# ntnu-arl/aerial_gym_simulator

Hardware: AMD Instinct MI355X
Metric: env-steps/sec at N_envs=8192 per GPU (dynamics-only) (higher is better)
Workload: dtype f32; 1 GPU; base_quadrotor position_setpoint_task, lee_position_control, empty_env, 1 sub-step/step (BASELINE configs[1]); num_envs_per_gpu=8192, num_envs_total=8192, rng=sync-free (device Philox4x32-10)

## Files before the change

aerial_gym_simulator_amd/csrc/agx_dyn_position_step.h:

```cpp
#pragma once

namespace agx {
#ifdef AGX_STEP_STAMPS
constexpr int kStampBlocks = 1024, kStampWords = 8;
__device__ unsigned long long g_step_stamps[kStampBlocks * 2 * kStampWords];
AGX_DEV void step_stamp(int k) {
  const unsigned long long t = k < 6 ? (unsigned long long)clock64() : (unsigned long long)wall_clock64();
  if ((threadIdx.x & 63u) == 0u && blockIdx.x < (unsigned)kStampBlocks)
    g_step_stamps[((size_t)blockIdx.x * 2 + (threadIdx.x >> 6)) * kStampWords + k] = t;
}
#define AGX_STAMP(k) step_stamp(k)
#define AGX_STAMP_ARRIVED(k) do { __builtin_amdgcn_s_waitcnt(0); step_stamp(k); } while (0)
#else
#define AGX_STAMP(k) do { } while (0)
#define AGX_STAMP_ARRIVED(k) do { } while (0)
#endif

AGX_DEV unsigned proof_key(float x) { return x >= 0.0f ? __float_as_uint(x) : 0x7FC00000u; }

__host__ __device__ inline unsigned proof_witness_bit(int episode_len, int reset_on_collision, int steps, float dist, float speed, float dt,
                                                      float vmax, float dv) {
  const int k = episode_len - steps + 1;
  if (k < 1 || k > AGX_PROOF_HORIZON || !(dist == dist) || !(speed == speed)) return 0u;
  bool w = k == 1 || !reset_on_collision;
  if (!w) {
    const float m = (float)(k - 1);
    const float travel = m * dt * fminf(vmax, speed + m * dv);
    w = dist + (travel * 1.01f + 1.0e-3f) < 8.0f;
  }
  return w ? (1u << k) : 0u;
}

template <bool MAX>
AGX_DEV unsigned wave_reduce_dpp(unsigned x) {
#define AGX_RED(ctrl)                                                                        \
  {                                                                                           \
    const unsigned y_ = (unsigned)__builtin_amdgcn_mov_dpp((int)x, (ctrl), 0xF, 0xF, true);   \
    x = MAX ? max(x, y_) : (x | y_);                                                          \
  }
  AGX_RED(0xB1)
  AGX_RED(0x4E)
  AGX_RED(0x124)
  AGX_RED(0x128)
#undef AGX_RED
  const unsigned r0 = (unsigned)__builtin_amdgcn_readlane((int)x, 0), r1 = (unsigned)__builtin_amdgcn_readlane((int)x, 16);
  const unsigned r2 = (unsigned)__builtin_amdgcn_readlane((int)x, 32), r3 = (unsigned)__builtin_amdgcn_readlane((int)x, 48);
  return MAX ? max(max(r0, r1), max(r2, r3)) : ((r0 | r1) | (r2 | r3));
}

AGX_DEV void proof_store_slot(const AgxTaskArgs &T, const AgxEnvBuffers &B, int wb, int nb, bool reset, unsigned horizon, int steps,
                              float dist, float speed) {
  const unsigned ar = wave_reduce_dpp<false>(reset ? 1u : 0u), hz = wave_reduce_dpp<false>(horizon);
  const unsigned ms = wave_reduce_dpp<true>((unsigned)max(steps, 0)), db = wave_reduce_dpp<true>(proof_key(dist));
  const unsigned vb = wave_reduce_dpp<true>(proof_key(speed));
  if ((threadIdx.x & 63u) == 0u) {
    uint4 *slot = reinterpret_cast<uint4 *>(T.proof_slots + ((size_t)(B.step_counter & 1) * nb + wb) * AGX_PROOF_SLOT_WORDS);
    slot[0] = make_uint4(((unsigned)B.step_counter + 1u) & 0x7FFFFFFFu, ar | (T.proof_mode == AGX_STEP_ANY ? 2u : 0u), hz, ms);
    slot[1] = make_uint4(db, vb, 0u, 0u);
  }
}

AGX_DEV void proof_fold_publish(const AgxTaskArgs &T, const AgxEnvBuffers &B, int nb) {
  const int lane = (int)(threadIdx.x & 63u);
  const uint32_t *bank = T.proof_slots + (size_t)((B.step_counter & 1) ^ 1) * nb * AGX_PROOF_SLOT_WORDS;
  unsigned t_and = 0x7FFFFFFFu, t_or = 0u, fl = 0u, hz = 0u, ms = 0u, db = 0u, vb = 0u;
  for (int b = lane; b < nb; b += 64) {
    const uint4 s0 = reinterpret_cast<const uint4 *>(bank + (size_t)b * AGX_PROOF_SLOT_WORDS)[0];
    const uint4 s1 = reinterpret_cast<const uint4 *>(bank + (size_t)b * AGX_PROOF_SLOT_WORDS)[1];
    t_and &= s0.x; t_or |= s0.x; fl |= s0.y; hz |= s0.z;
    ms = max(ms, s0.w); db = max(db, s1.x); vb = max(vb, s1.y);
  }
#pragma unroll
  for (int off = 32; off > 0; off >>= 1) {
    t_and &= (unsigned)__shfl_xor((int)t_and, off);
    t_or |= (unsigned)__shfl_xor((int)t_or, off);
    fl |= (unsigned)__shfl_xor((int)fl, off);
    hz |= (unsigned)__shfl_xor((int)hz, off);
    ms = max(ms, (unsigned)__shfl_xor((int)ms, off));
    db = max(db, (unsigned)__shfl_xor((int)db, off));
    vb = max(vb, (unsigned)__shfl_xor((int)vb, off));
  }
  if (lane != 0) return;
  const unsigned tag = t_and == t_or ? t_or : 0u;
  if (tag != 0u && (fl & 2u) && !(fl & 1u)) atomicAdd(T.proof_violation, 1u);
  uint32_t *h = T.proof_record;
  __hip_atomic_store(h + 7, tag, __ATOMIC_RELAXED, __HIP_MEMORY_SCOPE_SYSTEM);
  __builtin_amdgcn_fence(__ATOMIC_RELEASE, "wavefront");
  __builtin_amdgcn_s_waitcnt(0);
  __hip_atomic_store(h + 1, hz, __ATOMIC_RELAXED, __HIP_MEMORY_SCOPE_SYSTEM);
  __hip_atomic_store(h + 2, ms, __ATOMIC_RELAXED, __HIP_MEMORY_SCOPE_SYSTEM);
  __hip_atomic_store(h + 3, db, __ATOMIC_RELAXED, __HIP_MEMORY_SCOPE_SYSTEM);
  __hip_atomic_store(h + 4, vb, __ATOMIC_RELAXED, __HIP_MEMORY_SCOPE_SYSTEM);
  __hip_atomic_store(h + 5, fl, __ATOMIC_RELAXED, __HIP_MEMORY_SCOPE_SYSTEM);
  __builtin_amdgcn_fence(__ATOMIC_RELEASE, "wavefront");
  __builtin_amdgcn_s_waitcnt(0);
  __hip_atomic_store(h + 0, tag, __ATOMIC_RELAXED, __HIP_MEMORY_SCOPE_SYSTEM);
}

struct StepHandoff {
  float p[64], q[64], v[64], w[64];
  int reset[64];
};
template <int MODE>
AGX_DEV void position_step_quad(const AgxRobotParams &P0, const AgxEnvBuffers &B0, int n, const float *actions_in,
                                const AgxTaskArgs &T0, float *obs, StepHandoff *H) {
  constexpr bool FUSED = MODE != AGX_STEP_TWO;
  const int tid = threadIdx.x;
  AGX_STAMP(0); AGX_STAMP(6);
  AgxRobotParams P = P0;
  AgxEnvBuffers B = B0;
  AgxTaskArgs T = T0;
#define AGX_STEP_WAVE_ARGS(X)                                                                                                        \
  X(B, state) X(B, actions) X(B, prev_actions) X(B, motor_thrust) X(B, motor_kT) X(B, motor_tau_inc) X(B, motor_tau_dec)  \
  X(B, gains) X(B, wrench_cmd) X(B, crashes) X(B, truncations) X(B, sim_steps) X(B, reset_mask) X(B, reset_flag) X(B, flag_parity)    \
  X(B, step_counter) X(B, body_force)                                                                                                  \
  X(P, dt) X(P, dt_over_6) X(P, mass) X(P, min_thrust) X(P, max_thrust) X(P, max_rate) X(P, linear_damping) X(P, angular_damping)     \
  X(P, max_linear_velocity) X(P, max_angular_velocity) X(P, tau_inc_uniform) X(P, tau_dec_uniform)                                    \
  X(T, episode_len) X(T, target) X(T, reward) X(T, proof_slots) X(T, proof_violation) X(T, proof_dv)
  AGX_STEP_WAVE_ARGS(AGX_ARG_READ)
  AGX_ARG_READ(B, derived) AGX_ARG_READ(B, push_world)
  AGX_ARG_READ(P, root_link_mode) AGX_ARG_READ(P, use_rps) AGX_ARG_READ(P, use_discrete_approximation) AGX_ARG_READ(P, integration_rk4)
  AGX_ARG_READ(T, reset_on_collision) AGX_ARG_READ(T, kind) AGX_ARG_READ(T, proof_mode)
  const int grid_blocks = (int)gridDim.x;
  __builtin_amdgcn_sched_barrier(0);
  int env_blocks = grid_blocks - 1;
  int sw = (P_root_link_mode != 0 ? 1 : 0) | (P_use_rps != 0 ? 2 : 0) | (P_use_discrete_approximation != 0 ? 4 : 0) |
           (P_integration_rk4 != 0 ? 8 : 0) | (T_reset_on_collision != 0 ? 16 : 0) | ((T_kind & 0xFF) << 8) | ((T_proof_mode & 0xFF) << 16);
  arg_pin(n); arg_pin(actions_in);
  if (MODE == AGX_STEP_NONE) arg_pin(obs);
  AGX_STEP_WAVE_ARGS(AGX_ARG_PIN)
  if (MODE != AGX_STEP_ANY) { AGX_ARG_PIN(B, derived) }
  if (!FUSED) { AGX_ARG_PIN(B, push_world) }
  arg_pin(env_blocks);
#undef AGX_STEP_WAVE_ARGS
  arg_pin(sw);
  P.root_link_mode = sw & 1; P.use_rps = sw & 2; P.use_discrete_approximation = sw & 4; P.integration_rk4 = sw & 8;
  T.reset_on_collision = sw & 16; T.kind = (sw >> 8) & 0xFF; T.proof_mode = (sw >> 16) & 0xFF;
  const bool proof = T.proof_slots != nullptr;
  if (proof && blockIdx.x == 0) {
    proof_fold_publish(T0, B0, (int)gridDim.x - 1);
    AGX_STAMP(5); AGX_STAMP(7);
    return;
  }
  const int wb = (int)blockIdx.x - (proof ? 1 : 0);
  const int l = tid & 3, l3 = l < 3 ? l : 2;
  const int i = wb * 16 + (tid >> 2);
  const unsigned ol = ((unsigned)l * (unsigned)n + (unsigned)i) * 4u, ol3 = ((unsigned)l3 * (unsigned)n + (unsigned)i) * 4u;
  const bool valid = i < n;
  bool reset = false;
  if (FUSED && wb == 0 && tid == 0) B.reset_flag[B.flag_parity ^ 1] = 0;
  const bool push = !FUSED && wb == 0 && B.push_world > 0;
  uint32_t push_peek = 0u;
  if (__builtin_expect(push, false)) {
    push_publish_previous(B0);
    push_peek = push_wait_peek(B0);
  }
  float p = 0.0f, q = 0.0f, v = 0.0f, w = 0.0f, tgt = 0.0f, vbody = 0.0f, wbody = 0.0f;
  int steps = 0;
  float proof_dist = 0.0f, proof_speed = 0.0f;
  unsigned horizon = 0u;
  float u[1] = {0.0f}, a_in = 0.0f, a_old = 0.0f, fz = 0.0f, torque = 0.0f, dist = 0.0f;
  QuadDerived d{};
  bool crashed = false, trunc = false;
  AGX_STAMP(1);
  if (valid) {
    p = AGX_QAT(B.state, 0, ol3); q = AGX_QAT(B.state, 3, ol); v = AGX_QAT(B.state, 7, ol3); w = AGX_QAT(B.state, 10, ol3);
    u[0] = AGX_QAT(B.motor_thrust, 0, ol);
    float kT[1] = {1.0f}, tinc[1] = {P.tau_inc_uniform}, tdec[1] = {P.tau_dec_uniform};
    if (P.use_rps) kT[0] = AGX_QAT(B.motor_kT, 0, ol);
    if (B.motor_tau_inc) tinc[0] = AGX_QAT(B.motor_tau_inc, 0, ol);
    if (B.motor_tau_dec) tdec[0] = AGX_QAT(B.motor_tau_dec, 0, ol);
    a_in = actions_in[(size_t)i * 4 + l];
    a_old = AGX_QAT(B.actions, 0, ol);
    float kp = P0.gains_uniform[0 + l3], kv = P0.gains_uniform[3 + l3], kr = P0.gains_uniform[6 + l3], kw = P0.gains_uniform[9 + l3];
    if (B.gains) {
      kp = gain_load(&AGX_QAT(B.gains, 0, ol3)); kv = gain_load(&AGX_QAT(B.gains, 3, ol3));
      kr = gain_load(&AGX_QAT(B.gains, 6, ol3)); kw = gain_load(&AGX_QAT(B.gains, 9, ol3));
    }
    const int steps_in = B.sim_steps[i];
    tgt = T.kind == AGX_TASK_POSITION ? AGX_QAT(T.target, 0, ol3) : 0.0f;
    const QuadConsts<4> C = load_quad_consts<4>(P0, P, l, l3);
    AGX_STAMP_ARRIVED(2);

    const float a = clamp_minmax(a_in, -10.0f, 10.0f);
    float sy_sp, cy_sp;
    d = update_states_quad(q, v, w, q4::bc<3>(a), sy_sp, cy_sp);
    const float pe = a - p;
    const float ve = 0.0f - v;
    const float acc = kp * pe + kv * ve;
    const float f = (acc - C.grav) * C.mass;
    fz = quad_thrust_along_body_z(q, f, l);
    const float qd = quad_desired_orientation_pos_vel_sc(f, sy_sp, cy_sp, l);
    torque = quad_body_torque<true>(C, q, qd, d.wbody, 0.0f, kr, kw, l);

    float fb, tb;
    quad_allocate<4>(P, C, l == 2 ? fz : 0.0f, torque, u, kT, tinc, tdec, fb, tb);
    if (B.body_force && l < 3) AGX_QAT(B.body_force, 0, ol) = fb;
    quad_integrate(P, C, p, q, v, w, fb, tb, l);

    steps = steps_in + 1;
    if (T.kind == AGX_TASK_POSITION) {
      const float pe_t = q4::quat_apply(q4::conj(d.qveh), tgt - p);
      dist = q4::norm3(pe_t);
      if (dist > 8.0f) crashed = true;
      trunc = steps > T.episode_len;
      reset = (crashed && T.reset_on_collision) || trunc;
    }
  }
  AGX_STAMP(3);
  if (MODE == AGX_STEP_ANY) {
    H->p[tid] = p; H->q[tid] = q; H->v[tid] = v; H->w[tid] = w;
    H->reset[tid] = reset ? 1 : 0;
    __syncthreads();
  }
  AGX_STAMP(4);
  if (valid) {
    float rew = 0.0f;
    if (T.kind == AGX_TASK_POSITION) {
      const float ex = exp_cw((l == 0 ? -8.0f : -4.0f) * dist * dist);
      const float pos_reward = 3.0f * q4::bc<0>(ex) + 2.0f * q4::bc<1>(ex);
      const float dist_reward = (20.0f - dist) / 40.0f;
      const float axis_z = l == 2 ? 1.0f : 0.0f;
      const float up = q4::bc<2>(q4::quat_rotate(q, axis_z));
      const float tilt = fabsf(1.0f - up);
      const float spin = q4::norm3(d.wbody);
      const float quo = (1.0f / (l == 0 ? 0.1f + tilt * tilt : 1.0f + spin * spin)) * (l == 0 ? 0.2f : 3.0f);
      const float up_reward = q4::bc<0>(quo);
      const float ang_reward = q4::bc<1>(quo);
      float total = pos_reward + dist_reward + pos_reward * (up_reward + ang_reward);
      total = 1.0f * total;
      if (crashed) total = -20.0f;
      rew = total;
      proof_dist = dist;
    }
    if (proof) {
      proof_speed = q4::norm3(v);
      if (l == 0 && !reset && T.kind == AGX_TASK_POSITION) horizon = proof_witness_bit(T.episode_len, T.reset_on_collision, steps, proof_dist, proof_speed, P.dt, P.max_linear_velocity,
                                    T.proof_dv);
    }

    const bool own = MODE != AGX_STEP_ANY || !reset;
    if (own) {
      if (l < 3) AGX_QAT(B.state, 0, ol) = p;
      AGX_QAT(B.state, 3, ol) = q;
      if (l < 3) {
        AGX_QAT(B.state, 7, ol) = v;
        AGX_QAT(B.state, 10, ol) = w;
      }
      AGX_QAT(B.motor_thrust, 0, ol) = u[0];
    }
    if (MODE != AGX_STEP_ANY) {
      if (l < 3) {
        AGX_QAT(B.derived, 0, ol) = d.euler;
        AGX_QAT(B.derived, 7, ol) = d.vveh;
        AGX_QAT(B.derived, 10, ol) = d.vbody;
        AGX_QAT(B.derived, 13, ol) = d.wbody;
      }
      AGX_QAT(B.derived, 3, ol) = d.qveh;
    }
    vbody = d.vbody;
    wbody = d.wbody;
    if (B.wrench_cmd) {
      if (l < 3) {
        AGX_QAT(B.wrench_cmd, 0, ol) = l == 2 ? fz : 0.0f;
        AGX_QAT(B.wrench_cmd, 3, ol) = torque;
      }
    }
    AGX_QAT(B.prev_actions, 0, ol) = a_old;
    AGX_QAT(B.actions, 0, ol) = a_in;
    if (l == 0) {
      if (own) B.sim_steps[i] = steps;
      if (T.kind == AGX_TASK_POSITION) {
        T.reward[i] = rew;
        B.reset_mask[i] = reset ? 1 : 0;
      }
      B.crashes[i] = crashed ? 1 : 0;
      B.truncations[i] = trunc ? 1 : 0;
    }
  }
  const bool some = __ballot(reset) != 0ull;
  if (T.kind != AGX_TASK_NONE && some && (tid & 63) == 0) {
    atomicOr(B.reset_flag + B.flag_parity, 1);
    if (MODE == AGX_STEP_NONE) atomicAdd(T.proof_violation, 1u);
  }
  if (proof) proof_store_slot(T, B, wb, env_blocks, reset, horizon, steps, proof_dist, proof_speed);
  if (!FUSED) {
    if (__builtin_expect(push, false)) push_wait_finish(B0, push_peek);
    AGX_STAMP(5); AGX_STAMP(7);
    return;
  }
  if (MODE == AGX_STEP_ANY) {
    AGX_STAMP(5); AGX_STAMP(7);
    return;
  }
  if (valid) {
    float *o = obs + (size_t)i * 13;
    const float e = tgt - p;
    if (l < 3) { o[l] = e; o[7 + l] = vbody; o[10 + l] = wbody; }
    o[3 + l] = q;
  }
  AGX_STAMP(5); AGX_STAMP(7);
}

AGX_DEV void position_step_helper(const AgxRobotParams &P0, const AgxEnvBuffers &B0, int n, const AgxTaskArgs &T0, const AgxResetArgs &R0,
                                  float *obs, const StepHandoff *H) {
  AGX_STAMP(0); AGX_STAMP(6);
  AgxRobotParams P = P0;
  AgxEnvBuffers B = B0;
  AgxTaskArgs T = T0;
  AgxResetArgs R = R0;
#define AGX_HELPER_WAVE_ARGS(X, XN)                                                                                                  \
  X(B, sim_steps) X(B, episode_count) X(B, env_index_base) X(B, bounds_min) X(B, bounds_max) X(B, state) X(B, derived) X(B, gains)    \
  X(B, motor_tau_inc) X(B, motor_tau_dec) X(B, motor_thrust) X(B, motor_kT)                                                           \
  X(P, use_rps) X(P, min_thrust) X(P, max_thrust) X(T, kind) X(T, episode_len) X(T, target) X(T, proof_slots)                         \
  XN(R, lower_bound_min, 3) XN(R, lower_bound_max, 3) XN(R, upper_bound_min, 3) XN(R, upper_bound_max, 3) XN(R, min_state, 13)        \
  XN(R, max_state, 13) XN(R, gains_min, 12) XN(R, gains_max, 12) X(R, tau_inc_min) X(R, tau_inc_max) X(R, tau_dec_min)                \
  X(R, tau_dec_max) X(R, kT_min) X(R, kT_max) X(R, randomize_gains) X(R, seed)
  AGX_HELPER_WAVE_ARGS(AGX_ARG_READ, AGX_ARG_READ_N)
  arg_pin(n); arg_pin(obs);
  AGX_HELPER_WAVE_ARGS(AGX_ARG_PIN, AGX_ARG_PIN_N)
#undef AGX_HELPER_WAVE_ARGS
  const bool proof = T.proof_slots != nullptr;
  if (proof && blockIdx.x == 0) return;
  const int lane = (int)(threadIdx.x & 63u);
  const int wb = (int)blockIdx.x - (proof ? 1 : 0);
  const int l = lane & 3, l3 = l < 3 ? l : 2;
  const int i = wb * 16 + (lane >> 2);
  const unsigned ol = ((unsigned)l * (unsigned)n + (unsigned)i) * 4u, ol3 = ((unsigned)l3 * (unsigned)n + (unsigned)i) * 4u;
  const bool valid = i < n;
  int steps_in = 0, ep = 0;
  float tgt = 0.0f;
  AGX_STAMP(1);
  if (valid) {
    steps_in = B.sim_steps[i];
    if (B.episode_count) ep = B.episode_count[i];
    tgt = T.kind == AGX_TASK_POSITION ? AGX_QAT(T.target, 0, ol3) : 0.0f;
  }
  AGX_STAMP_ARRIVED(2);
  const bool early = valid && T.kind == AGX_TASK_POSITION && steps_in + 1 > T.episode_len;
  ResetValues<4> V{};
  if (vote(early) != 0ull) {
    ResetDraws<4> D{};
    wave_reset_draws<4>(R, B.env_index_base + i, ep, early && l == 0, D);
    V = reset_env_values<4>(P, R, D);
  }
  AGX_STAMP(3);
  __syncthreads();
  AGX_STAMP(4);
  float p = H->p[lane], q = H->q[lane], v = H->v[lane], w = H->w[lane];
  const bool mine = H->reset[lane] != 0;
  const bool late = mine && !early;
  if (vote(late) != 0ull) {
    ResetDraws<4> D{};
    wave_reset_draws<4>(R, B.env_index_base + i, ep, late && l == 0, D);
    const ResetValues<4> V2 = reset_env_values<4>(P, R, D);
    if (late) V = V2;
  }
  if (vote(mine) != 0ull) {
    if (mine && l == 0) reset_env_store<4>(P, B, n, R, i, ep, V);
    const EnvState &s = V.s;
    const float npv = q4::by_lane(l3, q4::bc<0>(s.p.x), q4::bc<0>(s.p.y), q4::bc<0>(s.p.z));
    const float nq = q4::by_lane(l, q4::bc<0>(s.q.x), q4::bc<0>(s.q.y), q4::bc<0>(s.q.z), q4::bc<0>(s.q.w));
    const float nv = q4::by_lane(l3, q4::bc<0>(s.v.x), q4::bc<0>(s.v.y), q4::bc<0>(s.v.z));
    const float nw = q4::by_lane(l3, q4::bc<0>(s.w.x), q4::bc<0>(s.w.y), q4::bc<0>(s.w.z));
    p = mine ? npv : p; q = mine ? nq : q; v = mine ? nv : v; w = mine ? nw : w;
  }
  const QuadDerived d2 = update_states_quad(q, v, w);
  if (valid) {
    if (l < 3) {
      AGX_QAT(B.derived, 0, ol) = d2.euler;
      AGX_QAT(B.derived, 7, ol) = d2.vveh;
      AGX_QAT(B.derived, 10, ol) = d2.vbody;
      AGX_QAT(B.derived, 13, ol) = d2.wbody;
    }
    AGX_QAT(B.derived, 3, ol) = d2.qveh;
    float *o = obs + (size_t)i * 13;
    const float e = tgt - p;
    if (l < 3) { o[l] = e; o[7 + l] = d2.vbody; o[10 + l] = d2.wbody; }
    o[3 + l] = q;
  }
  AGX_STAMP(5); AGX_STAMP(7);
}

__global__ void __launch_bounds__(64, 1)
    k_env_step_quad_position(AgxRobotParams P, AgxEnvBuffers B, int n, const float *__restrict__ actions_in, AgxTaskArgs T) {
  position_step_quad<AGX_STEP_TWO>(P, B, n, actions_in, T, nullptr, nullptr);
}

template <int MODE>
__global__ void __launch_bounds__(MODE == AGX_STEP_ANY ? 128 : 64, 1)
    k_position_step_fused(AgxRobotParams P, AgxEnvBuffers B, int n, const float *__restrict__ actions_in, AgxTaskArgs T, AgxResetArgs R,
                          float *__restrict__ obs) {
  if constexpr (MODE == AGX_STEP_ANY) {
    __shared__ StepHandoff H;
    if (__builtin_amdgcn_readfirstlane((int)(threadIdx.x >> 6)) == 0) position_step_quad<MODE>(P, B, n, actions_in, T, obs, &H);
    else position_step_helper(P, B, n, T, R, obs, &H);
  } else {
    position_step_quad<MODE>(P, B, n, actions_in, T, obs, nullptr);
  }
}

#ifdef AGX_STEP_STAMPS
}
extern "C" int agx_debug_step_stamps(unsigned long long *out, int blocks) {
  if (blocks < 0 || blocks > agx::kStampBlocks) return -1;
  return (int)hipMemcpyFromSymbol(out, HIP_SYMBOL(agx::g_step_stamps), sizeof(unsigned long long) * 2 * agx::kStampWords * (size_t)blocks);
}
namespace agx {
#endif
}

extern "C" float agx_step_proof_dv(const AgxRobotParams *P) {
  if (!P || !(P->mass > 0.0f)) return INFINITY;
  const int M = P->num_motors;
  const float *wmap = P->root_link_mode != 0 ? P->alloc : P->wrench_map;
  float col = 0.0f;
  for (int j = 0; j < M; ++j) col += sqrtf(wmap[j] * wmap[j] + wmap[M + j] * wmap[M + j] + wmap[2 * M + j] * wmap[2 * M + j]);
  const float g = sqrtf(P->gravity[0] * P->gravity[0] + P->gravity[1] * P->gravity[1] + P->gravity[2] * P->gravity[2]);
  return (col * fmaxf(fabsf(P->max_thrust), fabsf(P->min_thrust)) / P->mass + g) * P->dt * 1.1f;
}

extern "C" float agx_step_proof_travel(int m, float speed, float dt, float vmax, float dv, int per_env) {
  if (m <= 0) return 0.0f;
  float travel = 0.0f;
  if (per_env) {
    travel = (float)m * dt * fminf(vmax, speed + (float)m * dv);
  } else {
    float v = speed;
    for (int k = 0; k < m; ++k) {
      v = fminf(v + dv, vmax);
      travel += v * dt;
    }
  }
  return travel * 1.01f + 1.0e-3f;
}

extern "C" uint32_t agx_step_proof_witness_bit(int episode_len, int reset_on_collision, int steps, float dist, float speed, float dt,
                                               float max_linear_velocity, float dv) {
  return proof_witness_bit(episode_len, reset_on_collision, steps, dist, speed, dt, max_linear_velocity, dv);
}

extern "C" int agx_step_proof_decide(const uint32_t *record, const AgxStepProofQuery *q, int32_t *reason) {
  int32_t why = AGX_PROOF_PROVED;
  int mode = AGX_STEP_TWO;
  if (!record || !q) {
    why = AGX_PROOF_OFF;
  } else {
    volatile const uint32_t *h = record;
    const uint32_t end = h[0];
    __atomic_thread_fence(__ATOMIC_ACQUIRE);
    const uint32_t hz = h[1], ms = h[2], db = h[3], vb = h[4], fl = h[5];
    __atomic_thread_fence(__ATOMIC_ACQUIRE);
    const uint32_t begin = h[7];
    const uint32_t k = (q->now_tag - end) & 0x7FFFFFFFu;
    float dist, speed;
    memcpy(&dist, &db, 4);
    memcpy(&speed, &vb, 4);
    if (end != begin) why = AGX_PROOF_TORN;
    else if (end == 0u) why = AGX_PROOF_NO_RECORD;
    else if (((end - q->min_tag) & 0x7FFFFFFFu) >= 0x40000000u) why = AGX_PROOF_VOID;
    else if (k == 0u || k > 64u) why = AGX_PROOF_TAG;
    else if (k <= AGX_PROOF_HORIZON && ((hz >> k) & 1u)) mode = AGX_STEP_ANY;
    else if (fl & 1u) why = AGX_PROOF_RESET_NO_WITNESS;
    else if ((int64_t)ms + (int64_t)k > (int64_t)q->episode_len) why = AGX_PROOF_MAY_TRUNCATE;
    else if (q->reset_on_collision && (!(speed == speed) ||
                                       !(dist + agx_step_proof_travel((int)k, speed, q->dt, q->max_linear_velocity, q->dv, 0) < 8.0f)))
      why = AGX_PROOF_MAY_CRASH;
    else mode = AGX_STEP_NONE;
  }
  if (reason) *reason = why;
  return mode;
}

extern "C" int agx_host_record_alloc(size_t bytes, void **out) {
  AGX_REQUIRE(out && bytes > 0 && bytes <= (1u << 20), "bad arguments");
  void *p = nullptr;
  const hipError_t e = hipHostMalloc(&p, bytes, hipHostMallocMapped | hipHostMallocCoherent);
  if (e != hipSuccess) return fail(AGX_E_LAUNCH, "hipHostMalloc(%zu, mapped | coherent): %s", bytes, hipGetErrorString(e));
  memset(p, 0, bytes);
  *out = p;
  return AGX_OK;
}

extern "C" int agx_host_record_free(void *p) {
  if (p) (void)hipHostFree(p);
  return AGX_OK;
}

static int position_step_mode(AgxPositionStepPlan *plan, const AgxTaskArgs &T, hipStream_t stream, bool *slots, int32_t *reason) {
  *slots = false;
  const AgxEnvBuffers *B = plan->buf;
  const AgxRobotParams *P = plan->params;
  if (!option_single_launch_step() || !plan->proof_slots || !plan->proof_record || !plan->proof_violation) {
    *reason = AGX_PROOF_OFF;
    return AGX_STEP_TWO;
  }
  const bool covered = plan->k_substeps == 1 && pick_block(plan->num_envs) == 64 && P->num_motors == 4 &&
                       P->controller == AGX_CTRL_POSITION && T.kind == AGX_TASK_POSITION && quad_kernel_usable(P, B, &T) &&
                       plan->reset->u_state == nullptr && B->episode_count && !B->step_rows[0] && !B->step_rows[1] &&
                       !B->step_signal && B->push_world <= 0 && !B->step_counter_dev && plan->obs && plan->target == T.target;
  if (!covered) {
    *reason = AGX_PROOF_NOT_COVERED;
    return AGX_STEP_TWO;
  }
  if (!plan->captured) {
    hipStreamCaptureStatus cs = hipStreamCaptureStatusNone;
    if (hipStreamIsCapturing(stream, &cs) != hipSuccess || cs != hipStreamCaptureStatusNone) plan->captured = 1;
  }
  if (plan->captured) {
    *reason = AGX_PROOF_CAPTURE;
    return AGX_STEP_TWO;
  }
  *slots = true;
  const int max_lag = plan->max_lag > 0 ? plan->max_lag : 8;
  AgxStepProofQuery Q{};
  Q.now_tag = ((uint32_t)B->step_counter + 1u) & 0x7FFFFFFFu;
  Q.min_tag = plan->proof_min_tag;
  Q.episode_len = T.episode_len;
  Q.reset_on_collision = T.reset_on_collision;
  Q.dt = P->dt;
  Q.max_linear_velocity = P->max_linear_velocity;
  Q.dv = T.proof_dv;
  if (plan->slot_run > max_lag) {
    volatile const uint32_t *h = plan->proof_record;
    uint32_t k = (Q.now_tag - h[0]) & 0x7FFFFFFFu;
    if (h[0] != 0u && k > (uint32_t)max_lag && k <= 64u) {
      const auto t0 = std::chrono::steady_clock::now();
      const auto waited = [&] {
        plan->lag_waits += 1;
        plan->lag_wait_ns += (uint64_t)std::chrono::duration_cast<std::chrono::nanoseconds>(std::chrono::steady_clock::now() - t0).count();
      };
      for (unsigned spin = 1;; ++spin) {
        k = (Q.now_tag - h[0]) & 0x7FFFFFFFu;
        if (k <= (uint32_t)max_lag || k > 64u) break;
        __builtin_ia32_pause();
        if ((spin & 255u) == 0u && std::chrono::steady_clock::now() - t0 > std::chrono::microseconds(2000)) {
          waited();
          *reason = AGX_PROOF_LAG;
          return AGX_STEP_TWO;
        }
      }
      waited();
    }
  }
  return agx_step_proof_decide(plan->proof_record, &Q, reason);
}

extern "C" int agx_position_task_step(AgxPositionStepPlan *plan, const float *actions_in, void *stream) {
  AGX_REQUIRE(plan && plan->params && plan->buf && plan->task && plan->reset, "null plan member");
  AGX_REQUIRE(plan->max_lag == 0 || (plan->max_lag >= 2 && plan->max_lag < AGX_PROOF_HORIZON), "max_lag %d outside 2 .. %d (0: 8)",
              plan->max_lag, AGX_PROOF_HORIZON - 1);
  plan->buf->flag_parity ^= 1;
  if (plan->buf->push_world > 0)
    if (int e = agx_push_advance(plan->buf)) return e;
  AgxTaskArgs T = *plan->task;
  T.proof_slots = nullptr;
  T.proof_record = nullptr;
  T.proof_violation = nullptr;
  T.proof_mode = AGX_STEP_TWO;
  T.proof_dv = agx_step_proof_dv(plan->params);
  bool slots = false;
  int32_t why = AGX_PROOF_OFF;
  const int mode = position_step_mode(plan, T, (hipStream_t)stream, &slots, &why);
  plan->last_mode = mode;
  plan->last_reason = why;
  plan->mode_count[mode] += 1;
  plan->reason_count[why] += 1;
  plan->slot_run = slots ? plan->slot_run + 1 : 0;
  if (slots) {
    T.proof_slots = plan->proof_slots;
    T.proof_record = plan->proof_record;
    T.proof_violation = plan->proof_violation;
    T.proof_mode = mode;
  }
  if (mode != AGX_STEP_TWO) {
    const AgxEnvBuffers *B = plan->buf;
    const int n = plan->num_envs;
    if (int e = check_reset(plan->params, B, n, plan->reset)) return e;
    AGX_REQUIRE(actions_in && B->state && B->derived && B->actions && B->prev_actions && B->motor_thrust && B->crashes && B->truncations &&
                    B->sim_steps && T.target && T.reward,
                "null buffer");
    const dim3 grid(blocks_for(n, 16) + 1);
    if (mode == AGX_STEP_ANY)
      hipLaunchKernelGGL(k_position_step_fused<AGX_STEP_ANY>, grid, dim3(128), 0, (hipStream_t)stream, *plan->params, *B, n, actions_in, T,
                         *plan->reset, plan->obs);
    else
      hipLaunchKernelGGL(k_position_step_fused<AGX_STEP_NONE>, grid, dim3(64), 0, (hipStream_t)stream, *plan->params, *B, n, actions_in, T,
                         *plan->reset, plan->obs);
    return check_launch("agx_position_task_step");
  }
  if (int e = agx_env_step(plan->params, plan->buf, plan->num_envs, actions_in, plan->k_substeps, &T, stream)) return e;
  const uint32_t wait_seq = plan->buf->push_wait_seq;
  plan->buf->push_wait_seq = 0;
  const int rc = agx_post_step_position(plan->params, plan->buf, plan->num_envs, plan->reset, plan->target, plan->obs, stream);
  plan->buf->push_wait_seq = wait_seq;
  return rc;
}
```

aerial_gym_simulator_amd/csrc/agx_dyn_quad.h:

```cpp
#pragma once

namespace agx {
namespace q4 = quad;
AGX_DEV unsigned long long vote(bool p) { return __builtin_amdgcn_ballot_w64(p); }

struct QuadDerived {
  float euler, qveh, vveh, vbody, wbody;
};
AGX_DEV QuadDerived update_states_quad(float q, float v, float w, float extra, float &esn, float &ecs) {
  const int l = q4::lane_in_quad();
  QuadDerived d;
  const float e = q4::euler_xyz_0_2pi(q);
  d.euler = ssa(e);
  float sy, cy;
  const float half_yaw = (q4::bc<2>(e) * 1.0f) * 0.5f;
  sincos_bounded(l < 2 ? extra : half_yaw, sy, cy);
  esn = sy;
  ecs = cy;
  d.qveh = l == 2 ? sy : (l == 3 ? cy : 0.0f);
  d.vveh = q4::quat_rotate_inverse(d.qveh, v);
  d.vbody = q4::quat_rotate_inverse(q, v);
  d.wbody = q4::quat_rotate_inverse(q, w);
  return d;
}
AGX_DEV QuadDerived update_states_quad(float q, float v, float w) {
  float sn, cs;
  return update_states_quad(q, v, w, 0.0f, sn, cs);
}

template <int M>
struct QuadConsts {
  float grav, in0, in1, in2, ii0, ii1, ii2, pinv[M / 4][6], mapf[M], mapt[M], mass, dt;
};
template <int M>
AGX_DEV QuadConsts<M> load_quad_consts(const AgxRobotParams &P, const AgxRobotParams &S, int l, int l3) {
  QuadConsts<M> C;
  C.grav = P.gravity[l3];
  C.in0 = P.inertia[3 * l3 + 0]; C.in1 = P.inertia[3 * l3 + 1]; C.in2 = P.inertia[3 * l3 + 2];
  C.ii0 = P.inertia_inv[3 * l3 + 0]; C.ii1 = P.inertia_inv[3 * l3 + 1]; C.ii2 = P.inertia_inv[3 * l3 + 2];
#pragma unroll
  for (int h = 0; h < M / 4; ++h)
#pragma unroll
    for (int c = 0; c < 6; ++c) C.pinv[h][c] = P.alloc_pinv[6 * (l + 4 * h) + c];
  const float *wmap = S.root_link_mode != 0 ? P.alloc : P.wrench_map;
#pragma unroll
  for (int j = 0; j < M; ++j) {
    C.mapf[j] = wmap[M * l3 + j];
    C.mapt[j] = wmap[M * (3 + l3) + j];
  }
  C.mass = S.mass;
  C.dt = S.dt;
  return C;
}
template <int M>
AGX_DEV QuadConsts<M> load_quad_consts(const AgxRobotParams &P, int l, int l3) {
  return load_quad_consts<M>(P, P, l, l3);
}
AGX_DEV float quad_thrust_along_body_z(float q, float f, int l) {
  const float t1 = q * q4::bc<2>(q), t2 = q4::perm<1, 0, 2, 3>(q) * q4::bc<3>(q);
  const float c2a = 2.0f * (l == 1 ? t1 - t2 : t1 + t2);
  const float sqq = q * q;
  const float m22 = 1.0f - 2.0f * (q4::bc<0>(sqq) + q4::bc<1>(sqq));
  return q4::dot3(f, l == 2 ? m22 : c2a);
}
AGX_DEV float quad_desired_orientation_pos_vel_sc(float f, float sy, float cy, int l) {
  const float b3 = fdiv(f, q4::norm3(f));
  const float tmp = l == 0 ? cy : (l == 1 ? sy : 0.0f);
  const float cb = q4::cross3(b3, tmp);
  const float b2 = fdiv(cb, q4::norm3(cb));
  const float b1 = q4::cross3(b2, b3);
  return q4::rotmat_cols_to_quat(b1, b2, b3);
}
AGX_DEV float quad_desired_orientation_pos_vel(float f, float yaw, int l) {
  float sy, cy;
  sincos_bounded(yaw, sy, cy);
  return quad_desired_orientation_pos_vel_sc(f, sy, cy, l);
}
template <bool ZERO_RATE, int M>
AGX_DEV float quad_body_torque(const QuadConsts<M> &C, float q, float qd, float wb, float wsp, float kr, float kw, int l) {
  const float qe = q4::quat_mul(q4::conj(q), qd);
  const float pp = q4::rot1(qe) * q4::rot2(qe);
  const float pw = qe * q4::bc<3>(qe);
  const float mp = 2.0f * (pp + pw);
  const float mm = 2.0f * (pp - pw);
  const float rot_err = 0.5f * (l == 1 ? mm - mp : -(mp - mm));
  const float jw = (C.in0 * q4::bc<0>(wb) + C.in1 * q4::bc<1>(wb)) + C.in2 * q4::bc<2>(wb);
  const float ff = q4::cross3(wb, jw);
  const float we = ZERO_RATE ? wb : wb - q4::quat_rotate(qe, wsp);
  return ((-kr) * rot_err - kw * we) + ff;
}
template <int M>
AGX_DEV void quad_allocate(const AgxRobotParams &P, const QuadConsts<M> &C, float force, float torque, float (&u)[M / 4],
                           const float (&kT)[M / 4], const float (&tinc)[M / 4], const float (&tdec)[M / 4], float &fb, float &tb) {
  const float w0 = q4::bc<0>(force), w1 = q4::bc<1>(force), w2 = q4::bc<2>(force);
  const float w3 = q4::bc<0>(torque), w4 = q4::bc<1>(torque), w5 = q4::bc<2>(torque);
#pragma unroll
  for (int h = 0; h < M / 4; ++h) {
    float r = 0.0f;
    r += C.pinv[h][0] * w0;
    r += C.pinv[h][1] * w1;
    r += C.pinv[h][2] * w2;
    r += C.pinv[h][3] * w3;
    r += C.pinv[h][4] * w4;
    r += C.pinv[h][5] * w5;
    u[h] = motor_update(P, r, u[h], kT[h], tinc[h], tdec[h]);
  }
  fb = 0.0f;
  tb = 0.0f;
#pragma unroll
  for (int h = 0; h < M / 4; ++h) {
    const float u0 = q4::bc<0>(u[h]), u1 = q4::bc<1>(u[h]), u2 = q4::bc<2>(u[h]), u3 = q4::bc<3>(u[h]);
    fb += C.mapf[4 * h + 0] * u0; fb += C.mapf[4 * h + 1] * u1; fb += C.mapf[4 * h + 2] * u2; fb += C.mapf[4 * h + 3] * u3;
    tb += C.mapt[4 * h + 0] * u0; tb += C.mapt[4 * h + 1] * u1; tb += C.mapt[4 * h + 2] * u2; tb += C.mapt[4 * h + 3] * u3;
  }
}
template <int M>
AGX_DEV void quad_integrate(const AgxRobotParams &P, const QuadConsts<M> &C, float &p, float &q, float &v, float &w, float fb, float tb,
                            int l) {
  const float dt = C.dt;
  const float fw = q4::quat_rotate(q, fb);
  const float wbi = q4::quat_rotate_inverse(q, w);
  const float jwi = (C.in0 * q4::bc<0>(wbi) + C.in1 * q4::bc<1>(wbi)) + C.in2 * q4::bc<2>(wbi);
  const float rhs = tb - q4::cross3(wbi, jwi);
  const float dwb = (C.ii0 * q4::bc<0>(rhs) + C.ii1 * q4::bc<1>(rhs)) + C.ii2 * q4::bc<2>(rhs);
  const float wb_new = wbi + dt * dwb;
  float w_new = q4::quat_rotate(q, wb_new);
  float v_new = v + dt * fdiv(fw, C.mass);
  v_new = v_new + C.grav * dt;
  const float ml = fmaxf(1.0f - P.linear_damping * dt, 0.0f);
  const float ma = fmaxf(1.0f - P.angular_damping * dt, 0.0f);
  v_new = v_new * ml;
  w_new = w_new * ma;
  const float v2 = q4::dot3(v_new, v_new), w2 = q4::dot3(w_new, w_new);
  if (v2 > P.max_linear_velocity * P.max_linear_velocity) v_new = v_new * fdiv(P.max_linear_velocity, fsqrt(v2));
  if (w2 > P.max_angular_velocity * P.max_angular_velocity) w_new = w_new * fdiv(P.max_angular_velocity, fsqrt(w2));
  p = p + v_new * dt;
  const float wm2 = q4::dot3(w_new, w_new);
  if (wm2 != 0.0f) {
    const float wm = fsqrt(wm2);
    const float half = dt * wm * 0.5f;
    float sn, cs;
    sincos_bounded(half, sn, cs);
    const float sc = fdiv(sn, wm);
    const float x1 = w_new * sc;
    const float r3 = (x1 * q4::bc<3>(q) + q4::rot1(x1) * q4::rot2(q)) - q4::rot2(x1) * q4::rot1(q);
    const float xq = x1 * q;
    const float rw = (-q4::bc<0>(xq) - q4::bc<1>(xq)) - q4::bc<2>(xq);
    float rq = l == 3 ? rw : r3;
    rq += q * cs;
    const float nn = fsqrt(q4::dot4(rq, rq));
    q = fdiv(rq, nn);
  }
  v = v_new;
  w = w_new;
}

AGX_DEV float euler_rates_to_body_rates_quad(float euler, float rz) {
  const int l = q4::lane_in_quad();
  float sn, cs;
  sincos_bounded(euler, sn, cs);
  const float sr = q4::bc<0>(sn), cr = q4::bc<0>(cs), sp = q4::bc<1>(sn), cp = q4::bc<1>(cs);
  const float m0 = q4::by_lane(l, 1.0f, 0.0f, 0.0f);
  const float m1 = q4::by_lane(l, 0.0f, cr, -sr);
  const float m2 = q4::by_lane(l, -sp, sr * cp, cr * cp);
  return (m0 * 0.0f + m1 * 0.0f) + m2 * rz;
}
AGX_DEV float quat_from_euler_quad(float ang) {
  const int l = q4::lane_in_quad();
  float sn, cs;
  sincos_bounded(ang * 0.5f, sn, cs);
  const float sr = q4::bc<0>(sn), cr = q4::bc<0>(cs), sp = q4::bc<1>(sn), cp = q4::bc<1>(cs), sy = q4::bc<2>(sn), cy = q4::bc<2>(cs);
  const float a1 = l == 2 ? sy : cy, b1 = l == 0 ? sr : cr, c1 = l == 1 ? sp : cp;
  const float a2 = l == 2 ? cy : sy, b2 = l == 0 ? cr : sr, c2 = l == 1 ? cp : sp;
  const float t1 = a1 * b1 * c1, t2 = a2 * b2 * c2;
  return (l == 0 || l == 2) ? t1 - t2 : t1 + t2;
}

template <int CTRL, int M>
AGX_DEV void quad_controller(const AgxRobotParams &P, const QuadConsts<M> &C, float p, float q, float v, const QuadDerived &d, float a,
                             float a2, float kp, float kv, float kr, float kw, int l, float &force, float &torque) {
  const float yaw = q4::bc<2>(d.euler);
  float fz = 0.0f;
  if (CTRL == AGX_CTRL_FULLY_ACTUATED) {
    float nq = sqrtf(q4::dot4(a2, a2));
    nq = nq < 1e-9f ? 1e-9f : nq;
    const float qd = a2 / nq;
    const float acc = kp * (a - p) + kv * (0.0f - v);
    const float f = (acc - C.grav) * C.mass;
    force = q4::quat_rotate_inverse(q, f);
    torque = quad_body_torque<true>(C, q, qd, d.wbody, 0.0f, kr, kw, l);
    return;
  }
  if (CTRL == AGX_CTRL_POSITION || CTRL == AGX_CTRL_VELOCITY || CTRL == AGX_CTRL_VEL_STEERING) {
    float acc;
    if (CTRL == AGX_CTRL_POSITION) {
      acc = kp * (a - p) + kv * (0.0f - v);
    } else {
      const float sp_vel_w = q4::quat_rotate(d.qveh, a);
      acc = kp * (p - p) + kv * (sp_vel_w - v);
    }
    const float f = (acc - C.grav) * C.mass;
    fz = quad_thrust_along_body_z(q, f, l);
    const float qd = quad_desired_orientation_pos_vel(f, CTRL == AGX_CTRL_VELOCITY ? yaw : q4::bc<3>(a), l);
    if (CTRL == AGX_CTRL_POSITION) {
      torque = quad_body_torque<true>(C, q, qd, d.wbody, 0.0f, kr, kw, l);
    } else {
      float wsp = euler_rates_to_body_rates_quad(d.euler, CTRL == AGX_CTRL_VELOCITY ? q4::bc<3>(a) : 0.0f);
      if (l == 2) wsp = fminf(fmaxf(wsp, -P.max_yaw_rate), P.max_yaw_rate);
      torque = quad_body_torque<false>(C, q, qd, d.wbody, wsp, kr, kw, l);
    }
  } else if (CTRL == AGX_CTRL_ACCELERATION) {
    const float f = (a - C.grav) * C.mass;
    fz = quad_thrust_along_body_z(q, f, l);
    const float fx = q4::bc<0>(f), fy = q4::bc<1>(f), fzc = q4::bc<2>(f);
    const float num = q4::by_lane(l, -fy, fx, 0.0f);
    const float den = q4::by_lane(l, sqrtf(fzc * fzc + fx * fx), fzc, 1.0f);
    const float ang = atan2_cw(num, den);
    const float qd = quat_from_euler_quad(l == 2 ? yaw : ang);
    float wsp = euler_rates_to_body_rates_quad(d.euler, q4::bc<3>(a));
    if (l == 2) wsp = fminf(fmaxf(wsp, -P.max_yaw_rate), P.max_yaw_rate);
    torque = quad_body_torque<false>(C, q, qd, d.wbody, wsp, kr, kw, l);
  } else if (CTRL == AGX_CTRL_ATTITUDE) {
    const float g0 = P.gravity[0], g1 = P.gravity[1], g2 = P.gravity[2];
    fz = (q4::bc<0>(a) + 1.0f) * C.mass * norm(V3{g0, g1, g2});
    float wsp = euler_rates_to_body_rates_quad(d.euler, q4::bc<3>(a));
    if (l == 2) wsp = fminf(fmaxf(wsp, -P.max_yaw_rate), P.max_yaw_rate);
    const float qd = quat_from_euler_quad(q4::by_lane(l, q4::bc<1>(a), q4::bc<2>(a), yaw));
    torque = quad_body_torque<false>(C, q, qd, d.wbody, wsp, kr, kw, l);
  } else {
    fz = (q4::bc<0>(a) - P.gravity[2]) * C.mass;
    float wsp = q4::perm<1, 2, 3, 3>(a);
    if (l == 2) wsp = fminf(fmaxf(wsp, -P.max_yaw_rate), P.max_yaw_rate);
    torque = quad_body_torque<false>(C, q, q, d.wbody, wsp, kr, kw, l);
  }
  force = l == 2 ? fz : 0.0f;
}

template <int M, int CTRL>
__global__ void __launch_bounds__(64, 1)
    k_env_step_quad_loop(AgxRobotParams P, AgxEnvBuffers B, int n, const float *__restrict__ actions_in, int k, AgxTaskArgs T) {
  static_assert((M == 4 && CTRL >= AGX_CTRL_POSITION && CTRL <= AGX_CTRL_VEL_STEERING) ||
                    (M == 8 && (CTRL == AGX_CTRL_FULLY_ACTUATED || CTRL == AGX_CTRL_POSITION || CTRL == AGX_CTRL_VELOCITY)),
                "the six Lee laws of the quadrotor; the octarotor (two motors per lane) under its three laws: fully actuated, Lee "
                "position, Lee velocity (control/__init__.py:94-96)");
  constexpr bool FA = CTRL == AGX_CTRL_FULLY_ACTUATED;
  constexpr int A = FA ? 7 : 4;
  constexpr int MH = M / 4;
  extern __shared__ float traj[];
  const int tid = threadIdx.x;
  const int l = tid & 3, l3 = l < 3 ? l : 2, slot = tid >> 2;
  const int i = blockIdx.x * 16 + slot;
  const unsigned ol = ((unsigned)l * (unsigned)n + (unsigned)i) * 4u, ol3 = ((unsigned)l3 * (unsigned)n + (unsigned)i) * 4u;
  bool reset = false;
  if (blockIdx.x == 0) push_publish_previous(B);
  const uint32_t push_peek = blockIdx.x == 0 ? push_wait_peek(B) : 0u;
  if (i < n) {
    float p = AGX_QAT(B.state, 0, ol3), q = AGX_QAT(B.state, 3, ol), v = AGX_QAT(B.state, 7, ol3), w = AGX_QAT(B.state, 10, ol3);
    float u[MH], kT[MH], tinc[MH], tdec[MH];
#pragma unroll
    for (int h = 0; h < MH; ++h) {
      u[h] = AGX_QAT(B.motor_thrust, 4 * h, ol);
      kT[h] = P.use_rps ? AGX_QAT(B.motor_kT, 4 * h, ol) : 1.0f;
      tinc[h] = B.motor_tau_inc ? AGX_QAT(B.motor_tau_inc, 4 * h, ol) : P.tau_inc_uniform;
      tdec[h] = B.motor_tau_dec ? AGX_QAT(B.motor_tau_dec, 4 * h, ol) : P.tau_dec_uniform;
    }
    const float a_in = actions_in[(size_t)i * A + l];
    const float a_old = AGX_QAT(B.actions, 0, ol);
    const float a_in2 = FA ? actions_in[(size_t)i * A + 3 + l] : 0.0f;
    const float a_old2 = FA ? AGX_QAT(B.actions, 3, ol) : 0.0f;
    const float kp = B.gains ? AGX_QAT(B.gains, 0, ol3) : P.gains_uniform[0 + l3];
    const float kv = B.gains ? AGX_QAT(B.gains, 3, ol3) : P.gains_uniform[3 + l3];
    const float kr = B.gains ? AGX_QAT(B.gains, 6, ol3) : P.gains_uniform[6 + l3];
    const float kw = B.gains ? AGX_QAT(B.gains, 9, ol3) : P.gains_uniform[9 + l3];
    const QuadConsts<M> C = load_quad_consts<M>(P, l, l3);
    const int steps_in = B.sim_steps[i];
    const float tgt = T.kind != AGX_TASK_NONE ? AGX_QAT(T.target, 0, ol3) : 0.0f;
    const float ppe = (T.kind != AGX_TASK_NONE && T.kind != AGX_TASK_POSITION) ? AGX_QAT(T.pos_err, 0, ol3) : 0.0f;
    const float a_prev_in = k == 0 ? AGX_QAT(B.prev_actions, 0, ol) : 0.0f;
    const float a_prev_in2 = (FA && k == 0) ? AGX_QAT(B.prev_actions, 3, ol) : 0.0f;
    const float dmax = B.disturb_max[l3], dmax_t = B.disturb_max[3 + l3];
    const float a = clamp_minmax(a_in, -10.0f, 10.0f);
    const float a2 = clamp_minmax(a_in2, -10.0f, 10.0f);
    constexpr int kBoxBatch = M == 8 ? 12 : 16;
    struct BoxCull { float cx[kBoxBatch], cy[kBoxBatch], cz[kBoxBatch], rad[kBoxBatch]; };
    const int nb = (B.boxes && k > 0) ? B.num_boxes : 0;
    auto load_cull = [&](int b0, BoxCull &K) {
#pragma unroll
      for (int u = 0; u < kBoxBatch; ++u) {
        const int b = b0 + 4 * u;
        const float *bx = B.boxes + (size_t)(b < nb ? b : b0) * 11 * n + i;
        K.cx[u] = bx[0]; K.cy[u] = bx[(size_t)n]; K.cz[u] = bx[2 * (size_t)n]; K.rad[u] = bx[10 * (size_t)n];
      }
    };
    BoxCull cull0{};
    if (l < nb) load_cull(l, cull0);
    QuadDerived d{};
    float force = 0.0f, torque = 0.0f, fb = 0.0f;
    float tlo = p, thi = p;
    for (int sub = 0; sub < k; ++sub) {
      d = update_states_quad(q, v, w);
      quad_controller<CTRL>(P, C, p, q, v, d, a, a2, kp, kv, kr, kw, l, force, torque);
      float tb;
      quad_allocate<M>(P, C, force, torque, u, kT, tinc, tdec, fb, tb);
      if (B.disturb) {
        const float *dd = B.disturb + (size_t)sub * 7 * n + i;
        const float occ = dd[0];
        fb += ((dmax - (-dmax)) * dd[(size_t)(1 + l3) * n] + (-dmax)) * occ;
        tb += ((dmax_t - (-dmax_t)) * dd[(size_t)(4 + l3) * n] + (-dmax_t)) * occ;
      } else if (B.disturb_prob > 0.0f) {
        float ud[7];
        rng_fill<7>(B.rng_seed, B.env_index_base + i, agx::step_index(B), RNG_DISTURB + sub, ud);
        const float occ = ud[0] < B.disturb_prob ? 1.0f : 0.0f;
        fb += ((dmax - (-dmax)) * q4::by_lane(l3, ud[1], ud[2], ud[3]) + (-dmax)) * occ;
        tb += ((dmax_t - (-dmax_t)) * q4::by_lane(l3, ud[4], ud[5], ud[6]) + (-dmax_t)) * occ;
      }
      quad_integrate(P, C, p, q, v, w, fb, tb, l);
      if (B.boxes) {
        if (l < 3) traj[(sub * 3 + l) * 16 + slot] = p;
        if (sub == 0) { tlo = p; thi = p; }
        tlo = fminf(tlo, p);
        thi = fmaxf(thi, p);
      }
    }
    if (B.body_force && l < 3 && k > 0) AGX_QAT(B.body_force, 0, ol) = fb;
    bool crashed = false;
    if (B.boxes && k > 0) {
      const V3 lo = V3{q4::bc<0>(tlo), q4::bc<1>(tlo), q4::bc<2>(tlo)}, hi = V3{q4::bc<0>(thi), q4::bc<1>(thi), q4::bc<2>(thi)};
      const float rad = P.collision_radius, r2 = rad * rad;
      bool hit = false;
      auto test_batch = [&](int b0, const BoxCull &K) {
#pragma unroll
        for (int u = 0; u < kBoxBatch; ++u) {
          const int b = b0 + 4 * u;
          const V3 c = V3{K.cx[u], K.cy[u], K.cz[u]};
          const float reach = K.rad[u] + rad + 1.0e-3f;
          const float dx = fmaxf(fmaxf(lo.x - c.x, c.x - hi.x), 0.0f);
          const float dy = fmaxf(fmaxf(lo.y - c.y, c.y - hi.y), 0.0f);
          const float dz = fmaxf(fmaxf(lo.z - c.z, c.z - hi.z), 0.0f);
          if (b < nb && !(dx * dx + dy * dy + dz * dz > reach * reach)) {
            const float *bx = B.boxes + (size_t)b * 11 * n + i;
            const Q4 bq = Q4{bx[3 * (size_t)n], bx[4 * (size_t)n], bx[5 * (size_t)n], bx[6 * (size_t)n]};
            const V3 bh = V3{bx[7 * (size_t)n], bx[8 * (size_t)n], bx[9 * (size_t)n]};
            for (int sub = 0; sub < k; ++sub) {
              const V3 ps = V3{traj[(sub * 3 + 0) * 16 + slot], traj[(sub * 3 + 1) * 16 + slot], traj[(sub * 3 + 2) * 16 + slot]};
              hit = hit || sphere_hits_box(ps, c, bq, bh, r2);
            }
          }
        }
      };
      if (l < nb) test_batch(l, cull0);
      for (int b0 = l + 4 * kBoxBatch; b0 < nb; b0 += 4 * kBoxBatch) {
        BoxCull K;
        load_cull(b0, K);
        test_batch(b0, K);
      }
      crashed = ((vote(hit) >> (tid & 60)) & 0xFull) != 0ull;
    }
    if (l < 3) AGX_QAT(B.state, 0, ol) = p;
    AGX_QAT(B.state, 3, ol) = q;
    if (l < 3) {
      AGX_QAT(B.state, 7, ol) = v;
      AGX_QAT(B.state, 10, ol) = w;
    }
    if (k > 0) {
      if (l < 3) {
        AGX_QAT(B.derived, 0, ol) = d.euler;
        AGX_QAT(B.derived, 7, ol) = d.vveh;
        AGX_QAT(B.derived, 10, ol) = d.vbody;
        AGX_QAT(B.derived, 13, ol) = d.wbody;
      }
      AGX_QAT(B.derived, 3, ol) = d.qveh;
#pragma unroll
      for (int h = 0; h < MH; ++h) AGX_QAT(B.motor_thrust, 4 * h, ol) = u[h];
      if (B.wrench_cmd && l < 3) {
        AGX_QAT(B.wrench_cmd, 0, ol) = force;
        AGX_QAT(B.wrench_cmd, 3, ol) = torque;
      }
      if (!FA || l < 3) {
        AGX_QAT(B.prev_actions, 0, ol) = k >= 2 ? a_in : a_old;
        AGX_QAT(B.actions, 0, ol) = a_in;
      }
      if (FA) {
        AGX_QAT(B.prev_actions, 3, ol) = k >= 2 ? a_in2 : a_old2;
        AGX_QAT(B.actions, 3, ol) = a_in2;
      }
    }
    const float acur = k > 0 ? a_in : a_old;
    const float aprev = k >= 2 ? a_in : (k == 1 ? a_old : a_prev_in);
    const float acur3 = FA ? q4::bc<0>(k > 0 ? a_in2 : a_old2) : q4::bc<3>(acur);
    const float aprev3 = FA ? q4::bc<0>(k >= 2 ? a_in2 : (k == 1 ? a_old2 : a_prev_in2)) : q4::bc<3>(aprev);
    const int steps = steps_in + 1;
    bool trunc = false;
    float rew = 0.0f;
    if (T.kind != AGX_TASK_NONE) {
      if (T.kind == AGX_TASK_POSITION) {
        EnvState s;
        s.p = V3{q4::bc<0>(p), q4::bc<1>(p), q4::bc<2>(p)};
        s.q = Q4{q4::bc<0>(q), q4::bc<1>(q), q4::bc<2>(q), q4::bc<3>(q)};
        s.v = V3{0, 0, 0};
        s.w = V3{0, 0, 0};
        rew = reward_position(s, Q4{q4::bc<0>(d.qveh), q4::bc<1>(d.qveh), q4::bc<2>(d.qveh), q4::bc<3>(d.qveh)},
                              V3{q4::bc<0>(d.wbody), q4::bc<1>(d.wbody), q4::bc<2>(d.wbody)},
                              V3{q4::bc<0>(tgt), q4::bc<1>(tgt), q4::bc<2>(tgt)}, crashed);
      } else {
        const float pe = q4::quat_rotate_inverse(d.qveh, tgt - p);
        if (l < 3) {
          AGX_QAT(T.prev_pos_err, 0, ol) = ppe;
          AGX_QAT(T.pos_err, 0, ol) = pe;
        }
        rew = reward_navigation(T.rp, T.curriculum_progress, V3{q4::bc<0>(pe), q4::bc<1>(pe), q4::bc<2>(pe)},
                                V3{q4::bc<0>(ppe), q4::bc<1>(ppe), q4::bc<2>(ppe)}, q4::bc<0>(acur), q4::bc<2>(acur), acur3,
                                q4::bc<0>(aprev), q4::bc<2>(aprev), aprev3, crashed);
      }
      trunc = steps > T.episode_len;
      reset = (crashed && T.reset_on_collision) || trunc;
      if (T.successes)
        nav_bookkeeping_epilogue(T, i, l == 0, V3{q4::bc<0>(tgt), q4::bc<1>(tgt), q4::bc<2>(tgt)}, V3{q4::bc<0>(p), q4::bc<1>(p), q4::bc<2>(p)},
                                 crashed, trunc);
    }
    if (l == 0) {
      B.sim_steps[i] = steps;
      if (T.kind != AGX_TASK_NONE) {
        T.reward[i] = rew;
        B.reset_mask[i] = reset ? 1 : 0;
      }
      B.crashes[i] = crashed ? 1 : 0;
      B.truncations[i] = trunc ? 1 : 0;
    }
  }
  if (T.kind != AGX_TASK_NONE && __ballot(reset) != 0ull && (tid & 63) == 0) atomicOr(B.reset_flag + B.flag_parity, 1);
  if (blockIdx.x == 0) push_wait_finish(B, push_peek);
}
}
```

Measured before the change: 1.007 billion env-steps/s.

## Offload vehicle-frame yaw and reset decision to helper wave in two-wave step

In the two-wave (AGX_STEP_ANY) mode, the step wave no longer computes the full update_states (euler, vveh, vbody) or the distance/reset decision. The helper wave computes the vehicle-frame quaternion from the pre-step orientation while idle, and after the barrier both waves recompute the reset predicate from the shared qveh. This shortens the critical path of the step wave by moving the euler/atan work to the otherwise idle helper. In exchange it adds a noinline call, shared-memory traffic, and duplicated reset logic that must stay consistent between the waves.

```diff
diff --git a/aerial_gym_simulator_amd/csrc/agx_dyn_position_step.h b/aerial_gym_simulator_amd/csrc/agx_dyn_position_step.h
--- a/aerial_gym_simulator_amd/csrc/agx_dyn_position_step.h
+++ b/aerial_gym_simulator_amd/csrc/agx_dyn_position_step.h
@@ -99,8 +99,22 @@
 
 struct StepHandoff {
   float p[64], q[64], v[64], w[64];
-  int reset[64];
+  float qveh[64];
 };
+struct PositionResetSet {
+  float dist;
+  bool crashed, trunc, reset;
+};
+AGX_DEV PositionResetSet position_reset_set(int episode_len, int reset_on_collision, float qveh, float tgt, float p, int steps_in) {
+  PositionResetSet s;
+  const float pe_t = q4::quat_apply(q4::conj(qveh), tgt - p);
+  s.dist = q4::norm3(pe_t);
+  s.crashed = false;
+  if (s.dist > 8.0f) s.crashed = true;
+  s.trunc = steps_in + 1 > episode_len;
+  s.reset = (s.crashed && reset_on_collision) || s.trunc;
+  return s;
+}
 template <int MODE>
 AGX_DEV void position_step_quad(const AgxRobotParams &P0, const AgxEnvBuffers &B0, int n, const float *actions_in,
                                 const AgxTaskArgs &T0, float *obs, StepHandoff *H) {
@@ -162,6 +176,7 @@
   float u[1] = {0.0f}, a_in = 0.0f, a_old = 0.0f, fz = 0.0f, torque = 0.0f, dist = 0.0f;
   QuadDerived d{};
   bool crashed = false, trunc = false;
+  int steps_in = 0;
   AGX_STAMP(1);
   if (valid) {
     p = AGX_QAT(B.state, 0, ol3); q = AGX_QAT(B.state, 3, ol); v = AGX_QAT(B.state, 7, ol3); w = AGX_QAT(B.state, 10, ol3);
@@ -177,14 +192,21 @@
       kp = gain_load(&AGX_QAT(B.gains, 0, ol3)); kv = gain_load(&AGX_QAT(B.gains, 3, ol3));
       kr = gain_load(&AGX_QAT(B.gains, 6, ol3)); kw = gain_load(&AGX_QAT(B.gains, 9, ol3));
     }
-    const int steps_in = B.sim_steps[i];
+    steps_in = B.sim_steps[i];
     tgt = T.kind == AGX_TASK_POSITION ? AGX_QAT(T.target, 0, ol3) : 0.0f;
     const QuadConsts<4> C = load_quad_consts<4>(P0, P, l, l3);
     AGX_STAMP_ARRIVED(2);
 
     const float a = clamp_minmax(a_in, -10.0f, 10.0f);
     float sy_sp, cy_sp;
-    d = update_states_quad(q, v, w, q4::bc<3>(a), sy_sp, cy_sp);
+    if (MODE == AGX_STEP_ANY) {
+      const bool own_qveh = vote(T.kind == AGX_TASK_POSITION && steps_in + 1 > T.episode_len) != 0ull;
+      d.qveh = vehicle_frame_quat_quad(q, own_qveh, q4::bc<3>(a), sy_sp, cy_sp);
+      d.wbody = q4::quat_rotate_inverse(q, w);
+      if (own_qveh) H->qveh[tid] = d.qveh;
+    } else {
+      d = update_states_quad(q, v, w, q4::bc<3>(a), sy_sp, cy_sp);
+    }
     const float pe = a - p;
     const float ve = 0.0f - v;
     const float acc = kp * pe + kv * ve;
@@ -199,7 +221,7 @@
     quad_integrate(P, C, p, q, v, w, fb, tb, l);
 
     steps = steps_in + 1;
-    if (T.kind == AGX_TASK_POSITION) {
+    if (MODE != AGX_STEP_ANY && T.kind == AGX_TASK_POSITION) {
       const float pe_t = q4::quat_apply(q4::conj(d.qveh), tgt - p);
       dist = q4::norm3(pe_t);
       if (dist > 8.0f) crashed = true;
@@ -210,11 +232,14 @@
   AGX_STAMP(3);
   if (MODE == AGX_STEP_ANY) {
     H->p[tid] = p; H->q[tid] = q; H->v[tid] = v; H->w[tid] = w;
-    H->reset[tid] = reset ? 1 : 0;
     __syncthreads();
   }
   AGX_STAMP(4);
   if (valid) {
+    if (MODE == AGX_STEP_ANY && T.kind == AGX_TASK_POSITION) {
+      const PositionResetSet s = position_reset_set(T.episode_len, T.reset_on_collision, H->qveh[tid], tgt, p, steps_in);
+      dist = s.dist; crashed = s.crashed; trunc = s.trunc; reset = s.reset;
+    }
     float rew = 0.0f;
     if (T.kind == AGX_TASK_POSITION) {
       const float ex = exp_cw((l == 0 ? -8.0f : -4.0f) * dist * dist);
@@ -303,7 +328,7 @@
 }
 
 AGX_DEV void position_step_helper(const AgxRobotParams &P0, const AgxEnvBuffers &B0, int n, const AgxTaskArgs &T0, const AgxResetArgs &R0,
-                                  float *obs, const StepHandoff *H) {
+                                  float *obs, StepHandoff *H) {
   AGX_STAMP(0); AGX_STAMP(6);
   AgxRobotParams P = P0;
   AgxEnvBuffers B = B0;
@@ -312,7 +337,8 @@
 #define AGX_HELPER_WAVE_ARGS(X, XN)                                                                                                  \
   X(B, sim_steps) X(B, episode_count) X(B, env_index_base) X(B, bounds_min) X(B, bounds_max) X(B, state) X(B, derived) X(B, gains)    \
   X(B, motor_tau_inc) X(B, motor_tau_dec) X(B, motor_thrust) X(B, motor_kT)                                                           \
-  X(P, use_rps) X(P, min_thrust) X(P, max_thrust) X(T, kind) X(T, episode_len) X(T, target) X(T, proof_slots)                         \
+  X(P, use_rps) X(P, min_thrust) X(P, max_thrust) X(T, kind) X(T, episode_len) X(T, reset_on_collision) X(T, target)                  \
+  X(T, proof_slots)                                                                                                                   \
   XN(R, lower_bound_min, 3) XN(R, lower_bound_max, 3) XN(R, upper_bound_min, 3) XN(R, upper_bound_max, 3) XN(R, min_state, 13)        \
   XN(R, max_state, 13) XN(R, gains_min, 12) XN(R, gains_max, 12) X(R, tau_inc_min) X(R, tau_inc_max) X(R, tau_dec_min)                \
   X(R, tau_dec_max) X(R, kT_min) X(R, kT_max) X(R, randomize_gains) X(R, seed)
@@ -329,10 +355,11 @@
   const unsigned ol = ((unsigned)l * (unsigned)n + (unsigned)i) * 4u, ol3 = ((unsigned)l3 * (unsigned)n + (unsigned)i) * 4u;
   const bool valid = i < n;
   int steps_in = 0, ep = 0;
-  float tgt = 0.0f;
+  float tgt = 0.0f, q0 = 0.0f;
   AGX_STAMP(1);
   if (valid) {
     steps_in = B.sim_steps[i];
+    q0 = AGX_QAT(B.state, 3, ol);
     if (B.episode_count) ep = B.episode_count[i];
     tgt = T.kind == AGX_TASK_POSITION ? AGX_QAT(T.target, 0, ol3) : 0.0f;
   }
@@ -343,12 +370,15 @@
     ResetDraws<4> D{};
     wave_reset_draws<4>(R, B.env_index_base + i, ep, early && l == 0, D);
     V = reset_env_values<4>(P, R, D);
+  } else {
+    H->qveh[lane] = vehicle_frame_quat_quad(q0);
   }
   AGX_STAMP(3);
   __syncthreads();
   AGX_STAMP(4);
   float p = H->p[lane], q = H->q[lane], v = H->v[lane], w = H->w[lane];
-  const bool mine = H->reset[lane] != 0;
+  bool mine = false;
+  if (T.kind == AGX_TASK_POSITION) mine = valid && position_reset_set(T.episode_len, T.reset_on_collision, H->qveh[lane], tgt, p, steps_in).reset;
   const bool late = mine && !early;
   if (vote(late) != 0ull) {
     ResetDraws<4> D{};
diff --git a/aerial_gym_simulator_amd/csrc/agx_dyn_quad.h b/aerial_gym_simulator_amd/csrc/agx_dyn_quad.h
--- a/aerial_gym_simulator_amd/csrc/agx_dyn_quad.h
+++ b/aerial_gym_simulator_amd/csrc/agx_dyn_quad.h
@@ -26,6 +26,21 @@
 AGX_DEV QuadDerived update_states_quad(float q, float v, float w) {
   float sn, cs;
   return update_states_quad(q, v, w, 0.0f, sn, cs);
+}
+__device__ __attribute__((noinline)) float euler_xyz_0_2pi_shared(float q) { return q4::euler_xyz_0_2pi(q); }
+AGX_DEV float vehicle_frame_quat_quad(float q, bool own, float extra, float &esn, float &ecs) {
+  const int l = q4::lane_in_quad();
+  float half_yaw = 0.0f;
+  if (own) half_yaw = (q4::bc<2>(euler_xyz_0_2pi_shared(q)) * 1.0f) * 0.5f;
+  float sy, cy;
+  sincos_bounded(l < 2 ? extra : half_yaw, sy, cy);
+  esn = sy;
+  ecs = cy;
+  return l == 2 ? sy : (l == 3 ? cy : 0.0f);
+}
+AGX_DEV float vehicle_frame_quat_quad(float q) {
+  float sn, cs;
+  return vehicle_frame_quat_quad(q, true, 0.0f, sn, cs);
 }
 
 template <int M>
```

After: 957.1 million env-steps/s. 4.9% lower.
